# reczoo/FuxiCTR

Measured on NVIDIA H100. Metric: samples/sec DeepFM Criteo-shape train_step (fwd+bwd+clip+Adam), higher is better.
Workload: dtype f32 (3xTF32 tensor-core GEMMs, fp32 everything else)

## Files before the change

### fuxictr_b200/csrc/dense.cu

```cuda
#include "b2_common.cuh"
#include "adam_common.cuh"

namespace {
constexpr int BM = 64, BN = 64, BK = 16, TM = 4, TN = 4;
constexpr int PAD = 4;

struct GemmArgs {
  const float* a; int64_t a_rs, a_cs;
  const float* b; int64_t b_rs, b_cs;
  float* c; int64_t ldc;
  int64_t M, N, K;
  const float* bias; const float* mul; const float* add;
  int act; int beta; int k_per_split;
};

template <bool KCONTIG>
__device__ __forceinline__ void load_tile(const float* __restrict__ p, int64_t rs, int64_t cs,
                                          int64_t r0, int64_t k0, int64_t R, int64_t Kend,
                                          float (&v)[4], int t, bool vec_ok) {
  if (KCONTIG) {
    const int r = t >> 2, k4 = (t & 3) * 4;
    const int64_t rr = r0 + r, kk = k0 + k4;
    if (vec_ok && rr < R && kk + 3 < Kend) {
      const float4 q = __ldg(reinterpret_cast<const float4*>(p + rr * rs + kk));
      v[0] = q.x; v[1] = q.y; v[2] = q.z; v[3] = q.w;
    } else {
#pragma unroll
      for (int i = 0; i < 4; ++i)
        v[i] = (rr < R && kk + i < Kend) ? __ldg(p + rr * rs + (kk + i) * cs) : 0.f;
    }
  } else {
    const int k = t >> 4, r4 = (t & 15) * 4;
    const int64_t rr = r0 + r4, kk = k0 + k;
    if (vec_ok && kk < Kend && rr + 3 < R) {
      const float4 q = __ldg(reinterpret_cast<const float4*>(p + kk * cs + rr));
      v[0] = q.x; v[1] = q.y; v[2] = q.z; v[3] = q.w;
    } else {
#pragma unroll
      for (int i = 0; i < 4; ++i)
        v[i] = (kk < Kend && rr + i < R) ? __ldg(p + (rr + i) * rs + kk * cs) : 0.f;
    }
  }
}

template <bool KCONTIG>
__device__ __forceinline__ void store_tile(float (*s)[BM + PAD], const float (&v)[4], int t) {
  if (KCONTIG) {
    const int r = t >> 2, k4 = (t & 3) * 4;
#pragma unroll
    for (int i = 0; i < 4; ++i) s[k4 + i][r] = v[i];
  } else {
    const int k = t >> 4, r4 = (t & 15) * 4;
    *reinterpret_cast<float4*>(&s[k][r4]) = make_float4(v[0], v[1], v[2], v[3]);
  }
}

template <bool A_KC, bool B_KC>
__global__ void __launch_bounds__(256)
sgemm_kernel(const GemmArgs g, bool a_vec, bool b_vec) {
  __shared__ __align__(16) float As[2][BK][BM + PAD];
  __shared__ __align__(16) float Bs[2][BK][BN + PAD];
  const int t = threadIdx.x;
  const int tx = t & 15, ty = t >> 4;
  const int64_t m0 = (int64_t) blockIdx.y * BM, n0 = (int64_t) blockIdx.x * BN;
  const int64_t kbeg = (int64_t) blockIdx.z * g.k_per_split;
  const int64_t kend = min(g.K, kbeg + g.k_per_split);

  float acc[TM][TN];
#pragma unroll
  for (int i = 0; i < TM; ++i)
#pragma unroll
    for (int j = 0; j < TN; ++j) acc[i][j] = 0.f;

  float ra[4], rb[4];
  load_tile<A_KC>(g.a, g.a_rs, g.a_cs, m0, kbeg, g.M, kend, ra, t, a_vec);
  load_tile<B_KC>(g.b, g.b_cs, g.b_rs, n0, kbeg, g.N, kend, rb, t, b_vec);
  store_tile<A_KC>(As[0], ra, t);
  store_tile<B_KC>(Bs[0], rb, t);
  __syncthreads();

  int cur = 0;
  for (int64_t k0 = kbeg; k0 < kend; k0 += BK) {
    const bool more = (k0 + BK) < kend;
    if (more) {
      load_tile<A_KC>(g.a, g.a_rs, g.a_cs, m0, k0 + BK, g.M, kend, ra, t, a_vec);
      load_tile<B_KC>(g.b, g.b_cs, g.b_rs, n0, k0 + BK, g.N, kend, rb, t, b_vec);
    }
#pragma unroll
    for (int k = 0; k < BK; ++k) {
      const float4 av = *reinterpret_cast<const float4*>(&As[cur][k][ty * TM]);
      const float4 bv = *reinterpret_cast<const float4*>(&Bs[cur][k][tx * TN]);
      const float a4[4] = {av.x, av.y, av.z, av.w};
      const float b4[4] = {bv.x, bv.y, bv.z, bv.w};
#pragma unroll
      for (int i = 0; i < TM; ++i)
#pragma unroll
        for (int j = 0; j < TN; ++j) acc[i][j] = fmaf(a4[i], b4[j], acc[i][j]);
    }
    if (more) {
      store_tile<A_KC>(As[cur ^ 1], ra, t);
      store_tile<B_KC>(Bs[cur ^ 1], rb, t);
      __syncthreads();
      cur ^= 1;
    }
  }

  const bool split = gridDim.z > 1;
#pragma unroll
  for (int i = 0; i < TM; ++i) {
    const int64_t m = m0 + ty * TM + i;
    if (m >= g.M) continue;
#pragma unroll
    for (int j = 0; j < TN; ++j) {
      const int64_t n = n0 + tx * TN + j;
      if (n >= g.N) continue;
      float v = acc[i][j];
      if (g.bias != nullptr && blockIdx.z == 0) v += __ldg(g.bias + n);
      float* cp = g.c + m * g.ldc + n;
      if (split) {
        b2_red_add(cp, v);
        continue;
      }
      if (g.mul != nullptr) v *= __ldg(g.mul + m * g.ldc + n);
      if (g.add != nullptr) v += __ldg(g.add + m * g.ldc + n);
      if (g.act == B2_ACT_RELU) v = fmaxf(v, 0.f);
      else if (g.act == B2_ACT_SIGMOID) v = 1.f / (1.f + expf(-v));
      if (g.beta) v += *cp;
      *cp = v;
    }
  }
}

__global__ void zero_strided_kernel(float* c, int64_t M, int64_t N, int64_t ldc) {
  const int64_t total = M * N;
  for (int64_t i = (int64_t) blockIdx.x * blockDim.x + threadIdx.x; i < total;
       i += (int64_t) gridDim.x * blockDim.x)
    c[(i / N) * ldc + (i % N)] = 0.f;
}
}

extern "C" B2_API int b2_gemm_f32(const float* a, int64_t a_rs, int64_t a_cs, const float* b,
                           int64_t b_rs, int64_t b_cs, float* c, int64_t ldc, int64_t M,
                           int64_t N, int64_t K, const float* bias, int act, const float* mul,
                           const float* add, int beta_accumulate, void* stream) {
  B2_REQUIRE(a && b && c, "NULL operand");
  B2_REQUIRE(M >= 0 && N >= 0 && K >= 0 && ldc >= N, "bad shape M=%lld N=%lld K=%lld ldc=%lld",
             (long long) M, (long long) N, (long long) K, (long long) ldc);
  B2_REQUIRE(a_rs == 1 || a_cs == 1, "A must have a unit stride");
  B2_REQUIRE(b_rs == 1 || b_cs == 1, "B must have a unit stride");
  B2_REQUIRE(act >= B2_ACT_NONE && act <= B2_ACT_SIGMOID, "bad activation code %d", act);
  if (M == 0 || N == 0) return B2_OK;
  cudaStream_t st = (cudaStream_t) stream;
  GemmArgs g;
  g.a = a; g.a_rs = a_rs; g.a_cs = a_cs;
  g.b = b; g.b_rs = b_rs; g.b_cs = b_cs;
  g.c = c; g.ldc = ldc; g.M = M; g.N = N; g.K = K;
  g.bias = bias; g.mul = mul; g.add = add; g.act = act; g.beta = beta_accumulate ? 1 : 0;
  const bool a_kc = (a_cs == 1);
  const bool b_kc = (b_rs == 1);
  const bool a_vec = ((uintptr_t) a % 16 == 0) && ((a_kc ? a_rs : a_cs) % 4 == 0);
  const bool b_vec = ((uintptr_t) b % 16 == 0) && ((b_kc ? b_cs : b_rs) % 4 == 0);
  const int64_t tiles = b2_ceil_div(M, BM) * b2_ceil_div(N, BN);
  int splits = 1;
  const bool linear = (act == B2_ACT_NONE && mul == nullptr && add == nullptr);
  if (linear && tiles < 2 * B2_NUM_SMS && K >= 8 * BK) {
    splits = (int) b2_ceil_div(3 * B2_NUM_SMS, tiles);
    const int64_t max_splits = K / (4 * BK);
    if (splits > max_splits) splits = (int) max_splits;
    if (splits < 1) splits = 1;
  }
  int64_t k_per = b2_ceil_div(b2_ceil_div(K, splits), BK) * BK;
  if (k_per < BK) k_per = BK;
  splits = (int) b2_ceil_div(K > 0 ? K : 1, k_per);
  g.k_per_split = (int) k_per;
  if (splits > 1 && !g.beta) {
    const int64_t total = M * N;
    int zgrid = (int) (b2_ceil_div(total, 256) < 1184 ? b2_ceil_div(total, 256) : 1184);
    zero_strided_kernel<<<zgrid, 256, 0, st>>>(c, M, N, ldc);
  }
  dim3 grid((unsigned) b2_ceil_div(N, BN), (unsigned) b2_ceil_div(M, BM), (unsigned) splits);
  B2_REQUIRE(grid.y <= 65535, "M too large for this launch geometry");
  if (a_kc && b_kc) sgemm_kernel<true, true><<<grid, 256, 0, st>>>(g, a_vec, b_vec);
  else if (a_kc && !b_kc) sgemm_kernel<true, false><<<grid, 256, 0, st>>>(g, a_vec, b_vec);
  else if (!a_kc && b_kc) sgemm_kernel<false, true><<<grid, 256, 0, st>>>(g, a_vec, b_vec);
  else sgemm_kernel<false, false><<<grid, 256, 0, st>>>(g, a_vec, b_vec);
  B2_CUDA_LAUNCH_CHECK("b2_gemm_f32");
  return B2_OK;
}

__global__ void __launch_bounds__(256)
logit_bce_kernel(const float* __restrict__ t0, const float* __restrict__ t1,
                 const float* __restrict__ t2, const float* __restrict__ t3,
                 const float* __restrict__ label, int64_t batch, float* __restrict__ y_pred,
                 float* __restrict__ loss, float* __restrict__ glogit) {
  b2_pdl_wait();
  b2_pdl_trigger();
  __shared__ float red[32];
  const float inv_b = 1.f / (float) batch;
  float part = 0.f;
  for (int64_t i = (int64_t) blockIdx.x * blockDim.x + threadIdx.x; i < batch;
       i += (int64_t) gridDim.x * blockDim.x) {
    float z = __ldg(t0 + i);
    if (t1 != nullptr) z += __ldg(t1 + i);
    if (t2 != nullptr) z += __ldg(t2 + i);
    if (t3 != nullptr) z += __ldg(t3 + i);
    const float p = 1.f / (1.f + expf(-z));
    if (y_pred != nullptr) y_pred[i] = p;
    if (label != nullptr) {
      const float y = __ldg(label + i);
      const float lp = fmaxf(logf(p), -100.f), lq = fmaxf(log1pf(-p), -100.f);
      part += -(y * lp + (1.f - y) * lq);
      if (glogit != nullptr) {
        const float pq = (1.f - p) * p;
        glogit[i] = ((p - y) / fmaxf(pq, 1e-12f)) * inv_b * pq;
      }
    }
  }
  if (loss != nullptr) {
    const float t = b2_block_sum(part, red);
    if (threadIdx.x == 0) b2_red_add(loss, t * inv_b);
  }
}

extern "C" B2_API int b2_logit_bce_fwd(const float* t0, const float* t1, const float* t2,
                                const float* t3, const float* label, int64_t batch,
                                float* y_pred, float* loss, float* glogit, void* stream) {
  B2_REQUIRE(t0 != nullptr, "first logit term is NULL");
  B2_REQUIRE(batch >= 1, "batch must be >= 1");
  B2_REQUIRE(label != nullptr || (loss == nullptr && glogit == nullptr), "loss/glogit need labels");
  cudaStream_t st = (cudaStream_t) stream;
  if (loss != nullptr) {
    cudaError_t e = cudaMemsetAsync(loss, 0, sizeof(float), st);
    if (e != cudaSuccess) return b2_fail(B2_E_CUDA, "b2_logit_bce_fwd: memset: %s", cudaGetErrorString(e));
  }
  int64_t blocks = b2_ceil_div(batch, 256);
  if (blocks > B2_NUM_SMS * 4) blocks = B2_NUM_SMS * 4;
  B2_LAUNCH(logit_bce_kernel, (int) blocks, 256, 0, st, t0, t1, t2, t3, label, batch, y_pred, loss, glogit);
  B2_CUDA_LAUNCH_CHECK("b2_logit_bce_fwd");
  return B2_OK;
}

constexpr int SUMSQ_UNROLL = 4;

__global__ void __launch_bounds__(256)
sumsq_kernel(const float* __restrict__ g, int64_t n, float* __restrict__ out,
             const uint8_t* __restrict__ flags, int64_t nf4) {
  b2_pdl_wait();
  b2_pdl_trigger();
  __shared__ float red[32];
  float acc = 0.f;
  const int64_t n4 = n >> 2;
  const float4* g4 = reinterpret_cast<const float4*>(g);
  const int64_t stride = (int64_t) gridDim.x * blockDim.x;
  for (int64_t i = (int64_t) blockIdx.x * blockDim.x + threadIdx.x; i < n4; i += SUMSQ_UNROLL * stride) {
    float4 v[SUMSQ_UNROLL];
#pragma unroll
    for (int u = 0; u < SUMSQ_UNROLL; ++u) {
      const int64_t j = i + u * stride;
      v[u] = make_float4(0.f, 0.f, 0.f, 0.f);
      if (j < n4 && (j >= nf4 || flags[j >> 2] != 0)) v[u] = b2_ldg_stream(g4 + j);
    }
#pragma unroll
    for (int u = 0; u < SUMSQ_UNROLL; ++u)
      acc += (v[u].x * v[u].x + v[u].y * v[u].y) + (v[u].z * v[u].z + v[u].w * v[u].w);
  }
  if (blockIdx.x == 0 && threadIdx.x < (n & 3)) {
    const float v = g[(n4 << 2) + threadIdx.x];
    acc += v * v;
  }
  const float t = b2_block_sum(acc, red);
  if (threadIdx.x == 0) b2_red_add(out, t);
}

extern "C" B2_API int b2_sumsq_ex(const float* g, int64_t n, float* out, const uint8_t* flags, int64_t n_flagged,
                                  void* stream) {
  B2_REQUIRE(g && out, "NULL pointer");
  B2_REQUIRE(((uintptr_t) g % 16) == 0, "gradient arena must be 16-byte aligned");
  B2_REQUIRE(flags == nullptr || (n_flagged >= 0 && n_flagged <= n && n_flagged % 4 == 0),
             "n_flagged=%lld must be a multiple of 4 in [0, n=%lld]", (long long) n_flagged, (long long) n);
  if (n <= 0) return B2_OK;
  int64_t blocks = b2_ceil_div(n >> 2, 256 * 4);
  if (blocks > (int64_t) B2_NUM_SMS * 8) blocks = (int64_t) B2_NUM_SMS * 8;
  if (blocks < 1) blocks = 1;
  const int64_t nf4 = flags != nullptr ? n_flagged >> 2 : 0;
  B2_LAUNCH(sumsq_kernel, (int) blocks, 256, 0, (cudaStream_t) stream, g, n, out, flags, nf4);
  B2_CUDA_LAUNCH_CHECK("b2_sumsq");
  return B2_OK;
}

extern "C" B2_API int b2_sumsq(const float* g, int64_t n, float* out, void* stream) {
  return b2_sumsq_ex(g, n, out, nullptr, 0, stream);
}

__global__ void adam_sched_kernel(const int64_t* __restrict__ step_dev, double lr, double beta1, double beta2,
                                  B2AdamSched* __restrict__ sched, int64_t sched_len) {
  const int64_t t = *step_dev;
  if (t < 1 || t >= sched_len) return;
  const double bc1 = 1.0 - pow(beta1, (double) t);
  const double bc2 = 1.0 - pow(beta2, (double) t);
  sched[t] = make_float2((float) (lr / bc1), (float) (1.0 / sqrt(bc2)));
}

__device__ __forceinline__ void adam_step_scalars(int64_t t, double lr, double beta1, double beta2, float& step_size,
                                                  float& ibc2) {
  const double bc1 = 1.0 - pow(beta1, (double) t);
  const double bc2 = 1.0 - pow(beta2, (double) t);
  step_size = (float) (lr / bc1);
  ibc2 = (float) (1.0 / sqrt(bc2));
}

__device__ __forceinline__ B2AdamConst adam_const(double beta1, double beta2, float eps) {
  B2AdamConst c;
  c.w1 = (float) (1.0 - beta1);
  c.b2 = (float) beta2;
  c.w2 = (float) (1.0 - beta2);
  c.eps = eps;
  return c;
}

__global__ void __launch_bounds__(256)
adam_kernel(float* __restrict__ p, float* __restrict__ g, float* __restrict__ m,
            float* __restrict__ v, int64_t n, const float* __restrict__ sumsq, float max_norm,
            double lr, double beta1, double beta2, float eps, const int64_t* __restrict__ step_dev,
            int zero_grad, const B2AdamSched* __restrict__ sched, uint8_t* __restrict__ flags, int64_t nf4,
            int touched_only) {
  b2_pdl_wait();
  b2_pdl_trigger();
  __shared__ B2AdamConst sc;
  __shared__ float s_clip, s_step, s_ibc2;
  if (threadIdx.x == 0) {
    const int64_t t = *step_dev;
    float clip = 1.f;
    if (sumsq != nullptr) {
      const float total_norm = sqrtf(*sumsq);
      clip = fminf(max_norm / (total_norm + 1e-6f), 1.f);
    }
    s_clip = clip;
    sc = adam_const(beta1, beta2, eps);
    if (sched != nullptr) {
      const B2AdamSched e = sched[t];
      s_step = e.x;
      s_ibc2 = e.y;
    } else {
      adam_step_scalars(t, lr, beta1, beta2, s_step, s_ibc2);
    }
  }
  __syncthreads();
  const B2AdamConst c = sc;
  const float clip = s_clip, step_size = s_step, ibc2 = s_ibc2;
  const int64_t n4 = n >> 2;
  float4* p4 = reinterpret_cast<float4*>(p);
  float4* g4 = reinterpret_cast<float4*>(g);
  float4* m4 = reinterpret_cast<float4*>(m);
  float4* v4 = reinterpret_cast<float4*>(v);
  const int lane = threadIdx.x & 31;
  for (int64_t i0 = (int64_t) blockIdx.x * blockDim.x + (threadIdx.x & ~31); i0 < n4;
       i0 += (int64_t) gridDim.x * blockDim.x) {
    const int64_t i = i0 + lane;
    const bool flagged = i < nf4;
    const bool live = !flagged || flags[i >> 2] != 0;
    if (i0 < nf4) __syncwarp();
    if (i >= n4 || (touched_only && !live)) continue;
    float4 pp = p4[i], mm = m4[i], vv = v4[i];
    const float4 gg = live ? g4[i] : make_float4(0.f, 0.f, 0.f, 0.f);
    b2_adam_apply(pp.x, __fmul_rn(gg.x, clip), mm.x, vv.x, c, step_size, ibc2);
    b2_adam_apply(pp.y, __fmul_rn(gg.y, clip), mm.y, vv.y, c, step_size, ibc2);
    b2_adam_apply(pp.z, __fmul_rn(gg.z, clip), mm.z, vv.z, c, step_size, ibc2);
    b2_adam_apply(pp.w, __fmul_rn(gg.w, clip), mm.w, vv.w, c, step_size, ibc2);
    p4[i] = pp; m4[i] = mm; v4[i] = vv;
    if (zero_grad && (gg.x != 0.f || gg.y != 0.f || gg.z != 0.f || gg.w != 0.f)) g4[i] = make_float4(0.f, 0.f, 0.f, 0.f);
    if (zero_grad && flagged && live && (i & 3) == 0) flags[i >> 2] = 0;
  }
  if (blockIdx.x == 0 && threadIdx.x < (n & 3)) {
    const int64_t i = (n4 << 2) + threadIdx.x;
    float pp = p[i], mm = m[i], vv = v[i];
    b2_adam_apply(pp, __fmul_rn(g[i], clip), mm, vv, c, step_size, ibc2);
    p[i] = pp; m[i] = mm; v[i] = vv;
    if (zero_grad) g[i] = 0.f;
  }
}

extern "C" B2_API int b2_adam_step_ex(float* p, float* g, float* m, float* v, int64_t n,
                                      const float* sumsq, float max_norm, double lr, double beta1,
                                      double beta2, float eps, const int64_t* step_dev, int zero_grad,
                                      uint8_t* flags, int64_t n_flagged, void* stream) {
  B2_REQUIRE(p && g && m && v && step_dev, "NULL pointer");
  B2_REQUIRE((((uintptr_t) p | (uintptr_t) g | (uintptr_t) m | (uintptr_t) v) % 16) == 0,
             "arenas must be 16-byte aligned");
  B2_REQUIRE(flags == nullptr || (n_flagged >= 0 && n_flagged <= n && n_flagged % 4 == 0),
             "n_flagged=%lld must be a multiple of 4 in [0, n=%lld]", (long long) n_flagged, (long long) n);
  if (n <= 0) return B2_OK;
  int64_t blocks = b2_ceil_div(n >> 2, 256 * 2);
  if (blocks > (int64_t) B2_NUM_SMS * 8) blocks = (int64_t) B2_NUM_SMS * 8;
  if (blocks < 1) blocks = 1;
  const B2AdamSched* no_sched = nullptr;
  const int64_t nf4 = flags != nullptr ? n_flagged >> 2 : 0;
  B2_LAUNCH(adam_kernel, (int) blocks, 256, 0, (cudaStream_t) stream, p, g, m, v, n, sumsq, max_norm, lr, beta1, beta2,
            eps, step_dev, zero_grad, no_sched, flags, nf4, 0);
  B2_CUDA_LAUNCH_CHECK("b2_adam_step");
  return B2_OK;
}

extern "C" B2_API int b2_adam_step(float* p, float* g, float* m, float* v, int64_t n,
                            const float* sumsq, float max_norm, double lr, double beta1,
                            double beta2, float eps, const int64_t* step_dev, int zero_grad,
                            void* stream) {
  return b2_adam_step_ex(p, g, m, v, n, sumsq, max_norm, lr, beta1, beta2, eps, step_dev, zero_grad, nullptr, 0,
                         stream);
}

constexpr int UNTOUCHED_THREADS = 1024, UNTOUCHED_UNROLL = 2;

__device__ __forceinline__ float4 ld_no_l1(const float4* p) {
  float4 r;
  asm volatile("ld.global.L1::no_allocate.v4.f32 {%0,%1,%2,%3}, [%4];"
               : "=f"(r.x), "=f"(r.y), "=f"(r.z), "=f"(r.w)
               : "l"(p));
  return r;
}
__device__ __forceinline__ void st_evict_first(float4* p, const float4& v) {
  asm volatile("st.global.cs.v4.f32 [%0], {%1,%2,%3,%4};" ::"l"(p), "f"(v.x), "f"(v.y), "f"(v.z), "f"(v.w)
               : "memory");
}

__global__ void __launch_bounds__(UNTOUCHED_THREADS, 1)
adam_untouched_kernel(float* __restrict__ p, float* __restrict__ m, float* __restrict__ v, int64_t n4,
                      const uint8_t* __restrict__ flags, double lr, double beta1, double beta2, float eps,
                      const int64_t* __restrict__ step_dev) {
  b2_pdl_wait();
  __shared__ B2AdamConst sc;
  __shared__ float s_step, s_ibc2;
  if (threadIdx.x == 0) {
    sc = adam_const(beta1, beta2, eps);
    adam_step_scalars(*step_dev + 1, lr, beta1, beta2, s_step, s_ibc2);
  }
  __syncthreads();
  const B2AdamConst c = sc;
  const float step_size = s_step, ibc2 = s_ibc2;
  float4* p4 = reinterpret_cast<float4*>(p);
  float4* m4 = reinterpret_cast<float4*>(m);
  float4* v4 = reinterpret_cast<float4*>(v);
  const int64_t stride = (int64_t) gridDim.x * blockDim.x;
  for (int64_t i = (int64_t) blockIdx.x * blockDim.x + threadIdx.x; i < n4; i += UNTOUCHED_UNROLL * stride) {
    bool on[UNTOUCHED_UNROLL];
#pragma unroll
    for (int u = 0; u < UNTOUCHED_UNROLL; ++u) {
      const int64_t j = i + u * stride;
      on[u] = j < n4 && flags[j >> 2] == 0;
    }
    float4 pp[UNTOUCHED_UNROLL], mm[UNTOUCHED_UNROLL], vv[UNTOUCHED_UNROLL];
#pragma unroll
    for (int u = 0; u < UNTOUCHED_UNROLL; ++u) {
      if (!on[u]) continue;
      const int64_t j = i + u * stride;
      pp[u] = ld_no_l1(p4 + j); mm[u] = ld_no_l1(m4 + j); vv[u] = ld_no_l1(v4 + j);
    }
#pragma unroll
    for (int u = 0; u < UNTOUCHED_UNROLL; ++u) {
      if (!on[u]) continue;
      const int64_t j = i + u * stride;
      b2_adam_apply(pp[u].x, 0.f, mm[u].x, vv[u].x, c, step_size, ibc2);
      b2_adam_apply(pp[u].y, 0.f, mm[u].y, vv[u].y, c, step_size, ibc2);
      b2_adam_apply(pp[u].z, 0.f, mm[u].z, vv[u].z, c, step_size, ibc2);
      b2_adam_apply(pp[u].w, 0.f, mm[u].w, vv[u].w, c, step_size, ibc2);
      st_evict_first(p4 + j, pp[u]); st_evict_first(m4 + j, mm[u]); st_evict_first(v4 + j, vv[u]);
    }
  }
}

extern "C" B2_API int b2_adam_untouched(float* p, float* m, float* v, int64_t n, const uint8_t* flags, double lr,
                                        double beta1, double beta2, float eps, const int64_t* step_dev, int max_ctas,
                                        void* stream) {
  B2_REQUIRE(p && m && v && flags && step_dev, "NULL pointer");
  B2_REQUIRE((((uintptr_t) p | (uintptr_t) m | (uintptr_t) v) % 16) == 0, "arenas must be 16-byte aligned");
  B2_REQUIRE(n >= 0 && n % 4 == 0, "n=%lld must be a multiple of 4", (long long) n);
  B2_REQUIRE(max_ctas >= 1, "max_ctas=%d must be >= 1", max_ctas);
  if (n == 0) return B2_OK;
  const int64_t n4 = n >> 2;
  int64_t blocks = b2_ceil_div(n4, UNTOUCHED_THREADS * UNTOUCHED_UNROLL);
  if (blocks > max_ctas) blocks = max_ctas;
  B2_LAUNCH(adam_untouched_kernel, (int) blocks, UNTOUCHED_THREADS, 0, (cudaStream_t) stream, p, m, v, n4, flags, lr,
            beta1, beta2, eps, step_dev);
  B2_CUDA_LAUNCH_CHECK("b2_adam_untouched");
  return B2_OK;
}

extern "C" B2_API int b2_adam_touched(float* p, float* g, float* m, float* v, int64_t n, const float* sumsq,
                                      float max_norm, double lr, double beta1, double beta2, float eps,
                                      const int64_t* step_dev, uint8_t* flags, void* stream) {
  B2_REQUIRE(p && g && m && v && step_dev && flags, "NULL pointer");
  B2_REQUIRE((((uintptr_t) p | (uintptr_t) g | (uintptr_t) m | (uintptr_t) v) % 16) == 0,
             "arenas must be 16-byte aligned");
  B2_REQUIRE(n >= 0 && n % 4 == 0, "n=%lld must be a multiple of 4", (long long) n);
  if (n == 0) return B2_OK;
  int64_t blocks = b2_ceil_div(n >> 2, 256 * 2);
  if (blocks > (int64_t) B2_NUM_SMS * 8) blocks = (int64_t) B2_NUM_SMS * 8;
  const B2AdamSched* no_sched = nullptr;
  B2_LAUNCH(adam_kernel, (int) blocks, 256, 0, (cudaStream_t) stream, p, g, m, v, n, sumsq, max_norm, lr, beta1, beta2,
            eps, step_dev, 1, no_sched, flags, n >> 2, 1);
  B2_CUDA_LAUNCH_CHECK("b2_adam_touched");
  return B2_OK;
}

extern "C" B2_API int b2_adam_sched(const int64_t* step_dev, double lr, double beta1, double beta2, float* sched,
                                    int64_t sched_len, void* stream) {
  B2_REQUIRE(step_dev && sched && sched_len >= 2, "NULL pointer / empty schedule table");
  adam_sched_kernel<<<1, 1, 0, (cudaStream_t) stream>>>(step_dev, lr, beta1, beta2,
                                                        reinterpret_cast<B2AdamSched*>(sched), sched_len);
  B2_CUDA_LAUNCH_CHECK("b2_adam_sched");
  return B2_OK;
}

extern "C" B2_API int b2_adam_step_sched(float* p, float* g, float* m, float* v, int64_t n, const float* sumsq,
                                         float max_norm, double beta1, double beta2, float eps,
                                         const int64_t* step_dev, const float* sched, int zero_grad,
                                         void* stream) {
  B2_REQUIRE(p && g && m && v && step_dev && sched, "NULL pointer");
  B2_REQUIRE((((uintptr_t) p | (uintptr_t) g | (uintptr_t) m | (uintptr_t) v) % 16) == 0,
             "arenas must be 16-byte aligned");
  if (n <= 0) return B2_OK;
  int64_t blocks = b2_ceil_div(n >> 2, 256 * 2);
  if (blocks > (int64_t) B2_NUM_SMS * 8) blocks = (int64_t) B2_NUM_SMS * 8;
  if (blocks < 1) blocks = 1;
  const B2AdamSched* sched_tab = reinterpret_cast<const B2AdamSched*>(sched);
  B2_LAUNCH(adam_kernel, (int) blocks, 256, 0, (cudaStream_t) stream, p, g, m, v, n, sumsq, max_norm, 0.0, beta1, beta2,
            eps, step_dev, zero_grad, sched_tab, (uint8_t*) nullptr, (int64_t) 0, 0);
  B2_CUDA_LAUNCH_CHECK("b2_adam_step_sched");
  return B2_OK;
}
```

Measured before the change: 8.507 million.

## Compact touched-row flags into shared-memory lists for sparse sumsq and Adam

Sumsq and the touched-only Adam kernel no longer scan every flagged float4 and test its flag byte. Each block now handles 1024-flag spans: it loads flags 16 bytes at a time, builds a compact list of set flags in shared memory with a warp prefix scan, and visits only the listed gradient/param float4s. Touched Adam also clears the flags while compacting and uses streaming loads and stores. This adds block barriers and scan work per span, and the cost of the compaction is only repaid when the flags are sparse.

```diff
diff --git a/fuxictr_b200/csrc/dense.cu b/fuxictr_b200/csrc/dense.cu
--- a/fuxictr_b200/csrc/dense.cu
+++ b/fuxictr_b200/csrc/dense.cu
@@ -242,6 +242,59 @@
 
 constexpr int SUMSQ_UNROLL = 4;
 
+constexpr int SPAN = 1024;
+constexpr int SPAN_LOADERS = SPAN / 16;
+
+__device__ __forceinline__ uint32_t nonzero_bytes(uint32_t w) {
+  const uint32_t m = __vcmpne4(w, 0u) & 0x01010101u;
+  return (m | (m >> 7) | (m >> 14) | (m >> 21)) & 0xfu;
+}
+
+template <bool kClear>
+__device__ __forceinline__ int compact_span(uint8_t* flags, int64_t s0, int64_t ngran, uint16_t* list, int* wsum) {
+  const int lane = threadIdx.x & 31, warp = threadIdx.x >> 5;
+  uint32_t bits = 0;
+  __syncthreads();
+  if (threadIdx.x < SPAN_LOADERS) {
+    const int64_t k0 = s0 + 16 * threadIdx.x;
+    if (k0 + 16 <= ngran && ((uintptr_t) flags & 15) == 0) {
+      uint4* f = reinterpret_cast<uint4*>(flags + k0);
+      const uint4 w = kClear ? *f : __ldg(f);
+      bits = nonzero_bytes(w.x) | nonzero_bytes(w.y) << 4 | nonzero_bytes(w.z) << 8 | nonzero_bytes(w.w) << 12;
+      if (kClear && bits != 0) *f = make_uint4(0u, 0u, 0u, 0u);
+    } else {
+      for (int j = 0; j < 16 && k0 + j < ngran; ++j) {
+        if (flags[k0 + j] != 0) {
+          bits |= 1u << j;
+          if (kClear) flags[k0 + j] = 0;
+        }
+      }
+    }
+  }
+  const int cnt = __popc(bits);
+  int incl = cnt;
+#pragma unroll
+  for (int d = 1; d < 32; d <<= 1) {
+    const int y = __shfl_up_sync(0xffffffffu, incl, d);
+    if (lane >= d) incl += y;
+  }
+  if (lane == 31) wsum[warp] = incl;
+  __syncthreads();
+  int pos = incl - cnt, total = 0;
+  for (int w = 0; w < (int) (blockDim.x >> 5); ++w) {
+    const int s = wsum[w];
+    if (w < warp) pos += s;
+    total += s;
+  }
+  while (bits != 0) {
+    list[pos++] = (uint16_t) (16 * threadIdx.x + __ffs(bits) - 1);
+    bits &= bits - 1;
+  }
+  __syncthreads();
+  return total;
+}
+
+template <bool kSpans>
 __global__ void __launch_bounds__(256)
 sumsq_kernel(const float* __restrict__ g, int64_t n, float* __restrict__ out,
              const uint8_t* __restrict__ flags, int64_t nf4) {
@@ -251,14 +304,35 @@
   float acc = 0.f;
   const int64_t n4 = n >> 2;
   const float4* g4 = reinterpret_cast<const float4*>(g);
+  if constexpr (kSpans) {
+    constexpr int U = 8;
+    __shared__ uint16_t list[SPAN];
+    __shared__ int wsum[8];
+    const int64_t ngran = (nf4 + 3) >> 2, nspans = (ngran + SPAN - 1) / SPAN;
+    for (int64_t s = blockIdx.x; s < nspans; s += gridDim.x) {
+      const int64_t f0 = s * SPAN * 4;
+      const int tasks = 4 * compact_span<false>(const_cast<uint8_t*>(flags), s * SPAN, ngran, list, wsum);
+      for (int q0 = threadIdx.x; q0 < tasks; q0 += U * blockDim.x) {
+        float4 x[U];
+#pragma unroll
+        for (int u = 0; u < U; ++u) {
+          const int q = q0 + u * blockDim.x;
+          const int64_t f = q < tasks ? f0 + 4 * list[q >> 2] + (q & 3) : nf4;
+          x[u] = f < nf4 ? b2_ldg_stream(g4 + f) : make_float4(0.f, 0.f, 0.f, 0.f);
+        }
+#pragma unroll
+        for (int u = 0; u < U; ++u) acc += (x[u].x * x[u].x + x[u].y * x[u].y) + (x[u].z * x[u].z + x[u].w * x[u].w);
+      }
+    }
+  }
   const int64_t stride = (int64_t) gridDim.x * blockDim.x;
-  for (int64_t i = (int64_t) blockIdx.x * blockDim.x + threadIdx.x; i < n4; i += SUMSQ_UNROLL * stride) {
+  for (int64_t i = nf4 + (int64_t) blockIdx.x * blockDim.x + threadIdx.x; i < n4; i += SUMSQ_UNROLL * stride) {
     float4 v[SUMSQ_UNROLL];
 #pragma unroll
     for (int u = 0; u < SUMSQ_UNROLL; ++u) {
       const int64_t j = i + u * stride;
       v[u] = make_float4(0.f, 0.f, 0.f, 0.f);
-      if (j < n4 && (j >= nf4 || flags[j >> 2] != 0)) v[u] = b2_ldg_stream(g4 + j);
+      if (j < n4) v[u] = b2_ldg_stream(g4 + j);
     }
 #pragma unroll
     for (int u = 0; u < SUMSQ_UNROLL; ++u)
@@ -279,11 +353,16 @@
   B2_REQUIRE(flags == nullptr || (n_flagged >= 0 && n_flagged <= n && n_flagged % 4 == 0),
              "n_flagged=%lld must be a multiple of 4 in [0, n=%lld]", (long long) n_flagged, (long long) n);
   if (n <= 0) return B2_OK;
-  int64_t blocks = b2_ceil_div(n >> 2, 256 * 4);
+  const int64_t nf4 = flags != nullptr ? n_flagged >> 2 : 0;
+  const int64_t nspans = b2_ceil_div(b2_ceil_div(nf4, 4), SPAN);
+  int64_t blocks = b2_ceil_div((n >> 2) - nf4, 256 * 4);
+  if (blocks < nspans) blocks = nspans;
   if (blocks > (int64_t) B2_NUM_SMS * 8) blocks = (int64_t) B2_NUM_SMS * 8;
   if (blocks < 1) blocks = 1;
-  const int64_t nf4 = flags != nullptr ? n_flagged >> 2 : 0;
-  B2_LAUNCH(sumsq_kernel, (int) blocks, 256, 0, (cudaStream_t) stream, g, n, out, flags, nf4);
+  if (nf4 > 0)
+    B2_LAUNCH(sumsq_kernel<true>, (int) blocks, 256, 0, (cudaStream_t) stream, g, n, out, flags, nf4);
+  else
+    B2_LAUNCH(sumsq_kernel<false>, (int) blocks, 256, 0, (cudaStream_t) stream, g, n, out, flags, nf4);
   B2_CUDA_LAUNCH_CHECK("b2_sumsq");
   return B2_OK;
 }
@@ -318,12 +397,24 @@
   return c;
 }
 
+__device__ __forceinline__ float4 ld_no_l1(const float4* p) {
+  float4 r;
+  asm volatile("ld.global.L1::no_allocate.v4.f32 {%0,%1,%2,%3}, [%4];"
+               : "=f"(r.x), "=f"(r.y), "=f"(r.z), "=f"(r.w)
+               : "l"(p));
+  return r;
+}
+__device__ __forceinline__ void st_evict_first(float4* p, const float4& v) {
+  asm volatile("st.global.cs.v4.f32 [%0], {%1,%2,%3,%4};" ::"l"(p), "f"(v.x), "f"(v.y), "f"(v.z), "f"(v.w)
+               : "memory");
+}
+
+template <bool kSpans>
 __global__ void __launch_bounds__(256)
 adam_kernel(float* __restrict__ p, float* __restrict__ g, float* __restrict__ m,
             float* __restrict__ v, int64_t n, const float* __restrict__ sumsq, float max_norm,
             double lr, double beta1, double beta2, float eps, const int64_t* __restrict__ step_dev,
-            int zero_grad, const B2AdamSched* __restrict__ sched, uint8_t* __restrict__ flags, int64_t nf4,
-            int touched_only) {
+            int zero_grad, const B2AdamSched* __restrict__ sched, uint8_t* __restrict__ flags, int64_t nf4) {
   b2_pdl_wait();
   b2_pdl_trigger();
   __shared__ B2AdamConst sc;
@@ -353,6 +444,41 @@
   float4* g4 = reinterpret_cast<float4*>(g);
   float4* m4 = reinterpret_cast<float4*>(m);
   float4* v4 = reinterpret_cast<float4*>(v);
+  if constexpr (kSpans) {
+    constexpr int U = 4;
+    __shared__ uint16_t list[SPAN];
+    __shared__ int wsum[8];
+    const int64_t ngran = (nf4 + 3) >> 2, nspans = (ngran + SPAN - 1) / SPAN;
+    for (int64_t s = blockIdx.x; s < nspans; s += gridDim.x) {
+      const int64_t f0 = s * SPAN * 4;
+      const int tasks = 4 * compact_span<true>(flags, s * SPAN, ngran, list, wsum);
+      for (int q0 = threadIdx.x; q0 < tasks; q0 += U * blockDim.x) {
+        int64_t f[U];
+        float4 pp[U], gg[U], mm[U], vv[U];
+#pragma unroll
+        for (int u = 0; u < U; ++u) {
+          const int q = q0 + u * blockDim.x;
+          f[u] = q < tasks ? f0 + 4 * list[q >> 2] + (q & 3) : nf4;
+          if (f[u] < nf4) {
+            pp[u] = ld_no_l1(p4 + f[u]); gg[u] = ld_no_l1(g4 + f[u]);
+            mm[u] = ld_no_l1(m4 + f[u]); vv[u] = ld_no_l1(v4 + f[u]);
+          }
+        }
+#pragma unroll
+        for (int u = 0; u < U; ++u) {
+          if (f[u] >= nf4) continue;
+          b2_adam_apply(pp[u].x, __fmul_rn(gg[u].x, clip), mm[u].x, vv[u].x, c, step_size, ibc2);
+          b2_adam_apply(pp[u].y, __fmul_rn(gg[u].y, clip), mm[u].y, vv[u].y, c, step_size, ibc2);
+          b2_adam_apply(pp[u].z, __fmul_rn(gg[u].z, clip), mm[u].z, vv[u].z, c, step_size, ibc2);
+          b2_adam_apply(pp[u].w, __fmul_rn(gg[u].w, clip), mm[u].w, vv[u].w, c, step_size, ibc2);
+          p4[f[u]] = pp[u]; st_evict_first(m4 + f[u], mm[u]); st_evict_first(v4 + f[u], vv[u]);
+          if (gg[u].x != 0.f || gg[u].y != 0.f || gg[u].z != 0.f || gg[u].w != 0.f)
+            g4[f[u]] = make_float4(0.f, 0.f, 0.f, 0.f);
+        }
+      }
+    }
+    return;
+  }
   const int lane = threadIdx.x & 31;
   for (int64_t i0 = (int64_t) blockIdx.x * blockDim.x + (threadIdx.x & ~31); i0 < n4;
        i0 += (int64_t) gridDim.x * blockDim.x) {
@@ -360,7 +486,7 @@
     const bool flagged = i < nf4;
     const bool live = !flagged || flags[i >> 2] != 0;
     if (i0 < nf4) __syncwarp();
-    if (i >= n4 || (touched_only && !live)) continue;
+    if (i >= n4) continue;
     float4 pp = p4[i], mm = m4[i], vv = v4[i];
     const float4 gg = live ? g4[i] : make_float4(0.f, 0.f, 0.f, 0.f);
     b2_adam_apply(pp.x, __fmul_rn(gg.x, clip), mm.x, vv.x, c, step_size, ibc2);
@@ -395,8 +521,8 @@
   if (blocks < 1) blocks = 1;
   const B2AdamSched* no_sched = nullptr;
   const int64_t nf4 = flags != nullptr ? n_flagged >> 2 : 0;
-  B2_LAUNCH(adam_kernel, (int) blocks, 256, 0, (cudaStream_t) stream, p, g, m, v, n, sumsq, max_norm, lr, beta1, beta2,
-            eps, step_dev, zero_grad, no_sched, flags, nf4, 0);
+  B2_LAUNCH(adam_kernel<false>, (int) blocks, 256, 0, (cudaStream_t) stream, p, g, m, v, n, sumsq, max_norm, lr, beta1,
+            beta2, eps, step_dev, zero_grad, no_sched, flags, nf4);
   B2_CUDA_LAUNCH_CHECK("b2_adam_step");
   return B2_OK;
 }
@@ -411,17 +537,6 @@
 
 constexpr int UNTOUCHED_THREADS = 1024, UNTOUCHED_UNROLL = 2;
 
-__device__ __forceinline__ float4 ld_no_l1(const float4* p) {
-  float4 r;
-  asm volatile("ld.global.L1::no_allocate.v4.f32 {%0,%1,%2,%3}, [%4];"
-               : "=f"(r.x), "=f"(r.y), "=f"(r.z), "=f"(r.w)
-               : "l"(p));
-  return r;
-}
-__device__ __forceinline__ void st_evict_first(float4* p, const float4& v) {
-  asm volatile("st.global.cs.v4.f32 [%0], {%1,%2,%3,%4};" ::"l"(p), "f"(v.x), "f"(v.y), "f"(v.z), "f"(v.w)
-               : "memory");
-}
 
 __global__ void __launch_bounds__(UNTOUCHED_THREADS, 1)
 adam_untouched_kernel(float* __restrict__ p, float* __restrict__ m, float* __restrict__ v, int64_t n4,
@@ -493,11 +608,11 @@
              "arenas must be 16-byte aligned");
   B2_REQUIRE(n >= 0 && n % 4 == 0, "n=%lld must be a multiple of 4", (long long) n);
   if (n == 0) return B2_OK;
-  int64_t blocks = b2_ceil_div(n >> 2, 256 * 2);
+  int64_t blocks = b2_ceil_div(b2_ceil_div(n >> 2, 4), SPAN);
   if (blocks > (int64_t) B2_NUM_SMS * 8) blocks = (int64_t) B2_NUM_SMS * 8;
   const B2AdamSched* no_sched = nullptr;
-  B2_LAUNCH(adam_kernel, (int) blocks, 256, 0, (cudaStream_t) stream, p, g, m, v, n, sumsq, max_norm, lr, beta1, beta2,
-            eps, step_dev, 1, no_sched, flags, n >> 2, 1);
+  B2_LAUNCH(adam_kernel<true>, (int) blocks, 256, 0, (cudaStream_t) stream, p, g, m, v, n, sumsq, max_norm, lr, beta1,
+            beta2, eps, step_dev, 1, no_sched, flags, n >> 2);
   B2_CUDA_LAUNCH_CHECK("b2_adam_touched");
   return B2_OK;
 }
@@ -523,8 +638,8 @@
   if (blocks > (int64_t) B2_NUM_SMS * 8) blocks = (int64_t) B2_NUM_SMS * 8;
   if (blocks < 1) blocks = 1;
   const B2AdamSched* sched_tab = reinterpret_cast<const B2AdamSched*>(sched);
-  B2_LAUNCH(adam_kernel, (int) blocks, 256, 0, (cudaStream_t) stream, p, g, m, v, n, sumsq, max_norm, 0.0, beta1, beta2,
-            eps, step_dev, zero_grad, sched_tab, (uint8_t*) nullptr, (int64_t) 0, 0);
+  B2_LAUNCH(adam_kernel<false>, (int) blocks, 256, 0, (cudaStream_t) stream, p, g, m, v, n, sumsq, max_norm, 0.0, beta1,
+            beta2, eps, step_dev, zero_grad, sched_tab, (uint8_t*) nullptr, (int64_t) 0);
   B2_CUDA_LAUNCH_CHECK("b2_adam_step_sched");
   return B2_OK;
 }
```

New measurement: 8.536 million (median of 6 runs). No clear change (+0.3%).
